# ksalesin/mitsuba3-nasa

Measured on AMD Instinct MI355X. Metric: Msamples/s (pixels×spp/s) fwd + PRB grad, cornell_box 512²; 1/2/4/8 GPU, higher is better.
Workload: dtype f32; 1 GPU; cornell_box 512x512 @ 256 spp/GPU: path fwd (max_depth 8) + prb backward wrt 'white.reflectance.value'; film=512x512, spp_per_gpu=256, spp_total=256

## Files before the change

### mitsuba3-nasa_amd/csrc/mh_wavefront.hip

```cpp
#include <algorithm>
#include <cstdlib>
#include <cmath>
#include <cstring>

#include "mh_shading.hpp"

namespace mh {

struct WfState {
    uint32_t *pd[2];
    float *ox[2], *oy[2], *oz[2], *dx[2], *dy[2], *dz[2], *mt[2];
    float *bx[2], *by[2], *bz[2], *ppx[2], *ppy[2], *ppz[2], *ppdf[2];
    uint64_t *rng[2];
    float *lx[2], *ly[2], *lz[2];
    float *ht, *hu, *hv;
    uint32_t *hp, *hs;
    uint32_t *sid;
    float *sox, *soy, *soz, *sdx, *sdy, *sdz, *smt, *sax, *say, *saz, *sbx, *sby, *sbz;
};

constexpr uint32_t kSeg = 64;
#ifndef MH_SEG_XCD
#define MH_SEG_XCD 0
#endif
// ... 44 lines not shown
        }                                                                                             \
    } while (0)
#define MH_WF_DISPATCH_NR(K, NR, ...)                                                                 \
    do {                                                                                              \
        const dim3 g_(grid), b_(256);                                                                 \
        if (lds && packet) hipLaunchKernelGGL((K<true, true, NR, kEngBvh2>), g_, b_, sh, st, __VA_ARGS__);     \
        else if (lds) hipLaunchKernelGGL((K<true, false, NR, kEngBvh2>), g_, b_, sh, st, __VA_ARGS__);       \
        else if (packet) hipLaunchKernelGGL((K<false, true, NR, kEngBvh2>), g_, b_, sh, st, __VA_ARGS__);    \
        else switch (stream_engine(S)) {                                                              \
            case kEngQuant: hipLaunchKernelGGL((K<false, false, NR, kEngQuant>), g_, b_, sh, st, __VA_ARGS__); break; \
            case kEngWideC: hipLaunchKernelGGL((K<false, false, NR, kEngWideC>), g_, b_, sh, st, __VA_ARGS__); break; \
            case kEngWide: hipLaunchKernelGGL((K<false, false, NR, kEngWide>), g_, b_, sh, st, __VA_ARGS__); break;   \
            default: hipLaunchKernelGGL((K<false, false, NR, kEngBvh2>), g_, b_, sh, st, __VA_ARGS__); break;        \
        }                                                                                             \
    } while (0)

static inline size_t align_up(size_t x) { return (x + 255) & ~size_t(255); }

uint32_t wf_counter_words(uint32_t n_bounces) { return kCtrStride * (n_bounces + 1); }

#ifdef MH_DEBUG
hipError_t guard_read_wf(unsigned long long *out) {
    hipError_t e = hipMemcpyFromSymbol(out, HIP_SYMBOL(g_mh_guard), sizeof(g_mh_guard));
    const unsigned long long z[kGuardCount] = {};
    if (e == hipSuccess) e = hipMemcpyToSymbol(HIP_SYMBOL(g_mh_guard), z, sizeof(z));
    return e;
}
#endif
uint64_t wf_max_chunk() { return 1ull << kPidBits; }

size_t wf_workspace_bytes(uint64_t cap) {
    cap = (cap + kSeg - 1) / kSeg * kSeg;
    return 55 * align_up(cap * 4) + 2 * align_up(cap * 8);
}

static WfState carve(void *ws, uint64_t cap) {
    cap = (cap + kSeg - 1) / kSeg * kSeg;
    uint8_t *p = reinterpret_cast<uint8_t *>(ws);
    auto f = [&]() { float *r = reinterpret_cast<float *>(p); p += align_up(cap * 4); return r; };
    auto u = [&]() { uint32_t *r = reinterpret_cast<uint32_t *>(p); p += align_up(cap * 4); return r; };
    WfState w;
    for (int k = 0; k < 2; ++k) {
        w.pd[k] = u();
        w.ox[k] = f(); w.oy[k] = f(); w.oz[k] = f(); w.dx[k] = f(); w.dy[k] = f(); w.dz[k] = f(); w.mt[k] = f();
        w.bx[k] = f(); w.by[k] = f(); w.bz[k] = f(); w.ppx[k] = f(); w.ppy[k] = f(); w.ppz[k] = f(); w.ppdf[k] = f();
        w.lx[k] = f(); w.ly[k] = f(); w.lz[k] = f();
    }
    w.ht = f(); w.hu = f(); w.hv = f(); w.hp = u(); w.hs = u();
    w.sid = u();
    w.sox = f(); w.soy = f(); w.soz = f(); w.sdx = f(); w.sdy = f(); w.sdz = f(); w.smt = f();
    w.sax = f(); w.say = f(); w.saz = f(); w.sbx = f(); w.sby = f(); w.sbz = f();
    for (int k = 0; k < 2; ++k) {
        w.rng[k] = reinterpret_cast<uint64_t *>(p);
        p += align_up(cap * 8);
    }
    return w;
}

constexpr uint32_t kPkPlanes = 5, kPkExt = 3;
struct WfPacked {
    float4 *base, *ext;
    uint64_t stride;
    uint32_t *tea_base;
    uint64_t tstride;
    MH_DEV float4 *pl(int b, uint32_t k) const { return base + (uint64_t)(b * (int)kPkPlanes + (int)k) * stride; }
    MH_DEV float4 *ex(int b, uint32_t k) const { return ext + (uint64_t)(b * (int)kPkExt + (int)k) * stride; }
    MH_DEV uint32_t *tea(int b) const { return tea_base + (uint64_t)b * tstride; }
};
static WfPacked carve_packed(void *ws, void *ws_ext, uint64_t cap) {
    cap = (cap + kSeg - 1) / kSeg * kSeg;
    WfPacked p;
    p.stride = align_up(cap * 16) / 16;
    p.base = reinterpret_cast<float4 *>(ws);
    p.ext = reinterpret_cast<float4 *>(ws_ext);
    p.tea_base = reinterpret_cast<uint32_t *>(reinterpret_cast<uint8_t *>(ws) + 2 * kPkPlanes * align_up(cap * 16));
    p.tstride = align_up(cap * 4) / 4;
    return p;
}

MH_DEV uint32_t lane_id() { return threadIdx.x & 63u; }

#ifdef MH_EXP_BPHASE
__device__ unsigned long long g_bph[4][12];
#define MH_BPH_DECL uint64_t bph_t = __builtin_amdgcn_s_memtime(); uint64_t bph[12] = {0, 0, 0, 0, 0, 0, 0, 0, 0, 0, 0, 0};
#define MH_BPH(k) do { const uint64_t _t = __builtin_amdgcn_s_memtime(); bph[k] += _t - bph_t; bph_t = _t; } while (0)
#define MH_BPH_ITER() (bph[6] += 1)
#define MH_BPH_FLUSH(grp)                                                                 \
    do {                                                                                  \
        if (lane_id() == 0)                                                               \
            for (int _k = 0; _k < 12; ++_k) atomicAdd(&g_bph[grp][_k], (unsigned long long)bph[_k]); \
    } while (0)
#else
#define MH_BPH_DECL
#define MH_BPH(k) do {} while (0)
#define MH_BPH_ITER() do {} while (0)
#define MH_BPH_FLUSH(grp) do {} while (0)
#endif

struct SegIter {
    uint32_t seg, wave, nwaves;
};
MH_DEV SegIter seg_iter() {
    SegIter it;
#if MH_SEG_XCD
    it.seg = (blockIdx.x & 7u) * 8u + ((blockIdx.x >> 3) & 7u);
#else
    it.seg = blockIdx.x % kSeg;
#endif
    const uint32_t wpb = blockDim.x / 64u;
    it.wave = (blockIdx.x / kSeg) * wpb + threadIdx.x / 64u;
    it.nwaves = (gridDim.x / kSeg) * wpb;
    return it;
}
__host__ __device__ inline uint32_t seg_len(uint64_t n) { return (uint32_t)((n + kSeg - 1) / kSeg); }

MH_DEV uint32_t wave_append(uint32_t *count, bool pred) {
    const unsigned long long m = __ballot(pred);
    const uint32_t tot = (uint32_t)__popcll(m);
    uint32_t base = 0;
    if (lane_id() == 0 && tot) base = atomicAdd(count, tot);
    base = __builtin_amdgcn_readfirstlane(base);
    const uint32_t off = lane_rank(m);
    return base + off;
}

MH_DEV uint64_t pcg_inc(uint32_t seed_value, uint32_t lane) {
    uint32_t v0, v1;
    tea4(seed_value, lane, v0, v1);
    return ((uint64_t)v1 << 1) | 1u;
}

__global__ void __launch_bounds__(256)
k_wf_raygen(DScene S, LaneMap lm, uint32_t seed_value, uint64_t n, uint64_t plane, float *out,
            WfState w, uint32_t *ctr) {
    const uint64_t k = (uint64_t)blockIdx.x * blockDim.x + threadIdx.x;
    if (k < kSeg) {
        const uint64_t L = seg_len(n), b = k * L;
        ctr[k * 32] = b >= n ? 0u : (uint32_t)std::min<uint64_t>(L, n - b);
    }
    if (k >= n) return;
    uint32_t lane, px, py;
    lane_of(lm, k, lane, px, py);
    Pcg rng;
    rng.seed(seed_value, lane);
    float sx = (float)px + rng.next_float(), sy = (float)py + rng.next_float();
    RayT r = camera_ray(S, __builtin_fmaf(sx, S.inv_width, -0.f),
                        __builtin_fmaf(sy, S.inv_height, -0.f));
    w.pd[0][k] = (uint32_t)k;
    w.ox[0][k] = r.o.x; w.oy[0][k] = r.o.y; w.oz[0][k] = r.o.z;
    w.dx[0][k] = r.d.x; w.dy[0][k] = r.d.y; w.dz[0][k] = r.d.z; w.mt[0][k] = r.maxt;
    w.bx[0][k] = 1.f; w.by[0][k] = 1.f; w.bz[0][k] = 1.f;
    w.ppx[0][k] = 0.f; w.ppy[0][k] = 0.f; w.ppz[0][k] = 0.f; w.ppdf[0][k] = 1.f;
    w.rng[0][k] = rng.state;
    w.lx[0][k] = 0.f; w.ly[0][k] = 0.f; w.lz[0][k] = 0.f;
    out[k] = 0.f; out[plane + k] = 0.f; out[2 * plane + k] = 0.f;
    out[3 * plane + k] = sx; out[4 * plane + k] = sy;
}

MH_DEV bool block_has_stride_work(const SegIter &it, uint32_t n) {
    const uint32_t first_wave = (blockIdx.x / kSeg) * (blockDim.x / 64u);
    return first_wave * 64u < n;
}
MH_DEV bool block_has_range_work(const SegIter &it, uint32_t n) {
    const uint32_t first_wave = (blockIdx.x / kSeg) * (blockDim.x / 64u);
    const uint32_t per = (n + it.nwaves - 1) / it.nwaves;
    return first_wave * per < n;
// ... 707 lines not shown
            float rr_prob = fminf(beta_max * (eta * eta), 0.95f);
            bool rr_active = depth >= in.rr_depth;
            if (rr_active) beta = beta * rcp(rr_prob);
            bool rr_continue = rng.next_float() < rr_prob;
            active_next = active_next && (!rr_active || rr_continue);
            if (slot >= 0)
                add_slot(A, slot, prb_indirect_factor(active_next, si, to_local(si, ray.d), bsdf_weight, bs_pdf));
            if (si.valid) depth += 1;
            alive = active_next;
        }
        const uint32_t slot_n = sbase + wave_append(ctr_next + it.seg * 32, alive);
        const uint32_t sslot = sbase + wave_append(ctr + it.seg * 32 + 1, shadow);
        if (alive) {
            w.pd[nxt][slot_n] = pid | (depth << kPidBits);
            w.ox[nxt][slot_n] = ray.o.x; w.oy[nxt][slot_n] = ray.o.y; w.oz[nxt][slot_n] = ray.o.z;
            w.dx[nxt][slot_n] = ray.d.x; w.dy[nxt][slot_n] = ray.d.y; w.dz[nxt][slot_n] = ray.d.z;
            w.mt[nxt][slot_n] = ray.maxt;
            w.bx[nxt][slot_n] = beta.x; w.by[nxt][slot_n] = beta.y; w.bz[nxt][slot_n] = beta.z;
            w.ppx[nxt][slot_n] = prev_p.x; w.ppy[nxt][slot_n] = prev_p.y; w.ppz[nxt][slot_n] = prev_p.z;
            w.ppdf[nxt][slot_n] = prev_pdf;
            w.rng[nxt][slot_n] = rng.state;
            q.dl(nxt, 0)[slot_n] = dL.x; q.dl(nxt, 1)[slot_n] = dL.y; q.dl(nxt, 2)[slot_n] = dL.z;
#pragma unroll
            for (int kk = 0; kk < NR; ++kk)
                if ((uint32_t)kk < n_rgb) {
                    q.A(nxt, kk * 3 + 0)[slot_n] = A[kk][0];
                    q.A(nxt, kk * 3 + 1)[slot_n] = A[kk][1];
                    q.A(nxt, kk * 3 + 2)[slot_n] = A[kk][2];
                }
        }
        if (shadow) {
            w.sox[sslot] = sray.o.x; w.soy[sslot] = sray.o.y; w.soz[sslot] = sray.o.z;
            w.sdx[sslot] = sray.d.x; w.sdy[sslot] = sray.d.y; w.sdz[sslot] = sray.d.z; w.smt[sslot] = sray.maxt;
#pragma unroll
            for (int kk = 0; kk < NR; ++kk)
                if ((uint32_t)kk < n_rgb) {
                    q.G(kk * 3 + 0)[sslot] = G[kk][0];
                    q.G(kk * 3 + 1)[sslot] = G[kk][1];
                    q.G(kk * 3 + 2)[sslot] = G[kk][2];
                }
        }
    }
    flush_partial(acc, q);
}

struct PrbGen {
    uint64_t n_total;
    const float *grad_in;
    int coalesce;
};

struct WfBmp {
    float4 *fin;
    float4 *rec;
    uint32_t *mask[2];
    uint64_t stride;
    uint32_t n_depth;
    int32_t slot;
    MH_DEV float4 *r(uint32_t d, uint32_t k) const { return rec + (uint64_t)(d * 3u + k) * stride; }
};

size_t wf_bmp_workspace_bytes(uint64_t cap, uint32_t n_depth) {
    cap = (cap + kSeg - 1) / kSeg * kSeg;
    return (size_t)(2 + 3 * n_depth) * align_up(cap * 16) + 2 * align_up(cap * 4);
}

static WfBmp carve_bmp(void *ws, uint64_t cap, uint32_t n_depth, int32_t slot) {
    cap = (cap + kSeg - 1) / kSeg * kSeg;
    WfBmp b;
    b.stride = align_up(cap * 16) / 16;
    b.fin = reinterpret_cast<float4 *>(ws);
    b.rec = b.fin + 2 * b.stride;
    uint8_t *m = reinterpret_cast<uint8_t *>(b.rec + (uint64_t)3 * n_depth * b.stride);
    b.mask[0] = reinterpret_cast<uint32_t *>(m);
    b.mask[1] = reinterpret_cast<uint32_t *>(m + align_up(cap * 4));
    b.n_depth = n_depth;
    b.slot = slot;
    return b;
}

#ifndef MH_BOUNCE_BMP_WAVES
#define MH_BOUNCE_BMP_WAVES 4
#endif
template <int NR, bool Gen, bool Bm, bool Det>
__global__ void __launch_bounds__(256, Bm ? MH_BOUNCE_BMP_WAVES : MH_BOUNCE_PRB_WAVES)
k_wf_bounce_prb(DScene S0, IntegratorParams in, LaneMap lm, uint32_t seed_value, WfState w, WfPrb q,
                int cur, uint32_t seg_cap, uint32_t *ctr, uint32_t *ctr_next, PrbGen gen, WfBmp bm, WfDet det) {
    extern __shared__ uint4 lds[];
    const SegIter it = seg_iter();
    auto seg_count = [&](uint32_t sg) -> uint32_t {
        if (Gen) {
            const uint64_t b0 = (uint64_t)sg * seg_cap;
            return b0 >= gen.n_total ? 0u : (uint32_t)std::min<uint64_t>(seg_cap, gen.n_total - b0);
        }
        return __hip_atomic_load(ctr + sg * 32, __ATOMIC_RELAXED, __HIP_MEMORY_SCOPE_AGENT);
    };
    const uint32_t n = seg_count(it.seg);
    if (Gen && blockIdx.x < kSeg && threadIdx.x == 0) ctr[it.seg * 32] = n;
    if (!block_has_stride_work(it, n)) return;
    MH_BPH_DECL
    float *recs = reinterpret_cast<float *>(reinterpret_cast<uint8_t *>(lds) + fused_pairs_offset(S0));
    stage_pair_records(S0, recs);
    const DScene S = stage_tables(S0, lds);
    uint32_t *ws = reinterpret_cast<uint32_t *>(reinterpret_cast<uint8_t *>(lds) + S0.tab_bytes) +
                   (threadIdx.x >> 6) * S0.stack_size;
    uint8_t *dscr = reinterpret_cast<uint8_t *>(lds) + fused_scratch_offset(S0) + (threadIdx.x >> 6) * kDeferScratch;
    uint32_t n_shadow = 0;
    const int nxt = cur ^ 1;
    const uint32_t n_rgb = q.n_rgb;
    float acc[NR][3];
#pragma unroll
    for (int kk = 0; kk < NR; ++kk) acc[kk][0] = acc[kk][1] = acc[kk][2] = 0.f;
    MH_BPH(7);
    const uint32_t seg = it.seg;
    const uint32_t n_iter = (n + it.nwaves * 64u - 1) / (it.nwaves * 64u);
    for (uint32_t itr = 0; itr < n_iter; ++itr) {
        const uint32_t i = (itr * it.nwaves + it.wave) * 64u + lane_id();
        const uint32_t sbase = seg * seg_cap;
        MH_BPH_ITER();
        bool alive = false, shadow = false;
        uint32_t pid = 0, depth = 0;
        RayT ray{v3(0, 0, 0), v3(0, 0, 1), -1.f}, sray{v3(0, 0, 0), v3(0, 0, 1), -1.f};
        V3 beta, prev_p, dL;
        float prev_pdf = 1.f;
        float A[NR][3], G[NR][3];
        float Pp[NR][3];
#pragma unroll
        for (int kk = 0; kk < NR; ++kk) Pp[kk][0] = Pp[kk][1] = Pp[kk][2] = 0.f;
        Pcg rng;
        const uint32_t j = sbase + i;
        MH_GUARD(i >= n || i < seg_cap, kGuardQueueSlot);
        uint64_t gen_state = 0, gen_inc = 0;
        V3 Lrun = v3(0, 0, 0), Le_b = v3(0, 0, 0), Lr_pot = v3(0, 0, 0), D_pot = v3(0, 0, 0), q_ind = v3(0, 0, 0);
        float b_uvx = 0.f, b_uvy = 0.f;
        uint32_t vmask = 0, depth_v = 0;
        bool bvtx = false;
        if (i < n) {
            if (Gen) {
                pid = j;
                uint32_t lane, px, py;
                lane_of(lm, pid, lane, px, py);
                MH_GUARD(px < S0.width && py < S0.height, kGuardPixel);
                Pcg g;
                g.seed(seed_value, lane);
                const float sx = (float)px + g.next_float(), sy = (float)py + g.next_float();
                ray = camera_ray(S0, __builtin_fmaf(sx, S0.inv_width, -0.f),
                                 __builtin_fmaf(sy, S0.inv_height, -0.f));
                gen_state = g.state;
                gen_inc = g.inc;
                dL = gather_dL_wave_lds(S0, gen.coalesce, gen.grad_in, sx, sy, dscr);
            } else {
                const uint32_t pd = w.pd[cur][j];
                pid = pd & kPidMask;
                depth = pd >> kPidBits;
                ray.o = v3(w.ox[cur][j], w.oy[cur][j], w.oz[cur][j]);
                ray.d = v3(w.dx[cur][j], w.dy[cur][j], w.dz[cur][j]);
                ray.maxt = w.mt[cur][j];
            }
            MH_GUARD(pid < gen.n_total, kGuardPathId);
        }
        MH_BPH(0);
        const Hit h = packet_batch<false, true>(S0.nodes, S0.prims, S0.prim_pairs, S0.key_sp, ws, 1u, ray, i < n, recs, dscr);
        MH_BPH(1);
        if (i < n) {
            if (Gen) {
                beta = v3(1.f, 1.f, 1.f);
                prev_p = v3(0.f, 0.f, 0.f);
                prev_pdf = 1.f;
#pragma unroll
                for (int kk = 0; kk < NR; ++kk) A[kk][0] = A[kk][1] = A[kk][2] = 0.f;
                rng.state = gen_state;
            } else {
                const uint32_t jl = j;
                beta = v3(w.bx[cur][jl], w.by[cur][jl], w.bz[cur][jl]);
                prev_p = v3(w.ppx[cur][jl], w.ppy[cur][jl], w.ppz[cur][jl]);
                prev_pdf = w.ppdf[cur][jl];
                dL = v3(q.dl(cur, 0)[jl], q.dl(cur, 1)[jl], q.dl(cur, 2)[jl]);
#pragma unroll
                for (int kk = 0; kk < NR; ++kk)
#pragma unroll
                    for (int c = 0; c < 3; ++c) A[kk][c] = (uint32_t)kk < n_rgb ? q.A(cur, kk * 3 + c)[jl] : 0.f;
                rng.state = w.rng[cur][jl];
                if (Det) {
#pragma unroll
                    for (int kk = 0; kk < NR; ++kk)
#pragma unroll
                        for (int c = 0; c < 3; ++c) Pp[kk][c] = (uint32_t)kk < n_rgb ? det.P(cur, kk * 3 + c)[j] : 0.f;
                }
                if (Bm) {
                    Lrun = v3(w.lx[cur][j], w.ly[cur][j], w.lz[cur][j]);
// ... 41 lines not shown
            if (smooth) rho = tex_eval(S, S.bsdf_tex[b], si.uvx, si.uvy);
            const int32_t slot = smooth ? q.slot_of_tex[S.bsdf_tex[b]] : -1;
            if (Bm) {
                bvtx = slot >= (int32_t)kMaxRgbParams && depth < bm.n_depth;
                depth_v = depth | (bvtx ? (uint32_t)(slot - (int32_t)kMaxRgbParams) << 8 : 0u);
                b_uvx = si.uvx;
                b_uvy = si.uvy;
            }
            if (shadow) {
                V3 wo_em = to_local(si, ds.d);
                V3 bsdf_value_em;
                float bsdf_pdf_em;
                diffuse_eval_pdf(rho, si.wi, wo_em, true, bsdf_value_em, bsdf_pdf_em);
                float mis_em = ds.delta ? 1.f : mis_weight(ds.pdf, bsdf_pdf_em);
                V3 beta_mis_em = beta * mis_em;
                const V3 Lr = (beta_mis_em * bsdf_value_em) * em_weight;
                V3 dLe = dL * Lr;
#pragma unroll
                for (int kk = 0; kk < NR; ++kk) {
                    G[kk][0] = (dLe.x * (A[kk][0] * kInvPi));
                    G[kk][1] = (dLe.y * (A[kk][1] * kInvPi));
                    G[kk][2] = (dLe.z * (A[kk][2] * kInvPi));
                }
                if (slot >= 0 && si.wi.z > 0.f && wo_em.z > 0.f)
                    add_slot(G, slot, (((dL * em_weight) * beta_mis_em) * wo_em.z) * kInvPi);
                if (Bm) {
                    Lr_pot = Lr;
                    if (bvtx && si.wi.z > 0.f && wo_em.z > 0.f)
                        D_pot = (((dL * em_weight) * beta_mis_em) * wo_em.z) * kInvPi;
                }
            }

            (void)rng.next_float();
            float s2x = rng.next_float(), s2y = rng.next_float();
            V3 bs_wo = v3(0, 0, 0), bsdf_weight = v3(0, 0, 0);
            float bs_pdf = 0.f;
            if (smooth && active_next) {
                bs_wo = square_to_cosine_hemisphere(s2x, s2y);
                bs_pdf = kInvPi * bs_wo.z;
                bsdf_weight = (si.wi.z > 0.f && bs_pdf > 0.f) ? rho : v3(0, 0, 0);
            }
            ray = spawn_ray(si.p, si.n, to_world(si, bs_wo));
            beta = beta * bsdf_weight;
            prev_p = si.p;
            prev_pdf = bs_pdf;
            float beta_max = hmax(beta);
            active_next = active_next && beta_max != 0.f;
            float rr_prob = fminf(beta_max * (eta * eta), 0.95f);
            bool rr_active = depth >= in.rr_depth;
            if (rr_active) beta = beta * rcp(rr_prob);
            bool rr_continue = rng.next_float() < rr_prob;
            active_next = active_next && (!rr_active || rr_continue);
            if (slot >= 0) {
                const V3 c = prb_indirect_factor(active_next, si, to_local(si, ray.d), bsdf_weight, bs_pdf);
                add_slot(A, slot, c);
                if (Bm && bvtx) q_ind = c;
            }
            if (si.valid) depth += 1;
            alive = active_next;
        }
        MH_BPH(2);
        const uint32_t slot_n = sbase + wave_append(ctr_next + seg * 32, alive);
        MH_GUARD(!alive || slot_n - sbase < seg_cap, kGuardAppendSlot);
        if (alive) {
            w.pd[nxt][slot_n] = pid | (depth << kPidBits);
            w.ox[nxt][slot_n] = ray.o.x; w.oy[nxt][slot_n] = ray.o.y; w.oz[nxt][slot_n] = ray.o.z;
            w.dx[nxt][slot_n] = ray.d.x; w.dy[nxt][slot_n] = ray.d.y; w.dz[nxt][slot_n] = ray.d.z;
            w.mt[nxt][slot_n] = ray.maxt;
            w.bx[nxt][slot_n] = beta.x; w.by[nxt][slot_n] = beta.y; w.bz[nxt][slot_n] = beta.z;
            w.ppx[nxt][slot_n] = prev_p.x; w.ppy[nxt][slot_n] = prev_p.y; w.ppz[nxt][slot_n] = prev_p.z;
            w.ppdf[nxt][slot_n] = prev_pdf;
            w.rng[nxt][slot_n] = rng.state;
            q.tea(nxt)[slot_n] = (uint32_t)(rng.inc >> 1);
            q.dl(nxt, 0)[slot_n] = dL.x; q.dl(nxt, 1)[slot_n] = dL.y; q.dl(nxt, 2)[slot_n] = dL.z;
#pragma unroll
            for (int kk = 0; kk < NR; ++kk)
                if ((uint32_t)kk < n_rgb) {
                    q.A(nxt, kk * 3 + 0)[slot_n] = A[kk][0];
                    q.A(nxt, kk * 3 + 1)[slot_n] = A[kk][1];
                    q.A(nxt, kk * 3 + 2)[slot_n] = A[kk][2];
                }
        }
        MH_BPH(3);
        const Hit sh = packet_batch<true, true, Gen>(S0.nodes, S0.prims, S0.prim_pairs, S0.key_sp, ws, 1u, sray, shadow, recs, dscr);
        MH_BPH(4);
        const bool unocc = shadow && sh.shape == MH_INVALID;
        if (unocc) {
            float (&ga)[NR][3] = Det ? Pp : acc;
#pragma unroll
            for (int kk = 0; kk < NR; ++kk)
                if ((uint32_t)kk < n_rgb) {
                    ga[kk][0] += G[kk][0];
                    ga[kk][1] += G[kk][1];
                    ga[kk][2] += G[kk][2];
                }
        }
        if (Det && i < n) {
#pragma unroll
            for (int kk = 0; kk < NR; ++kk)
                if ((uint32_t)kk < n_rgb)
#pragma unroll
                    for (int c = 0; c < 3; ++c) {
                        if (alive) det.P(nxt, kk * 3 + c)[slot_n] = Pp[kk][c];
                        else det.fin(kk * 3 + c)[pid] = Pp[kk][c];
                    }
        }
        if (Bm && i < n) {
            Lrun = (Lrun + Le_b) + (unocc ? Lr_pot : v3(0, 0, 0));
            const V3 D = unocc ? D_pot : v3(0, 0, 0);
            if (bvtx && (nonzero(q_ind) || nonzero(D))) {
                const uint32_t dv = depth_v & 0xffu;
                bm.r(dv, 0)[pid] = make_float4(Lrun.x, Lrun.y, Lrun.z, b_uvx);
                bm.r(dv, 1)[pid] = make_float4(q_ind.x, q_ind.y, q_ind.z, b_uvy);
                bm.r(dv, 2)[pid] = make_float4(D.x, D.y, D.z, __uint_as_float(depth_v >> 8));
                vmask |= 1u << dv;
            }
            if (alive) {
                w.lx[nxt][slot_n] = Lrun.x; w.ly[nxt][slot_n] = Lrun.y; w.lz[nxt][slot_n] = Lrun.z;
                bm.mask[nxt][slot_n] = vmask;
            } else {
                bm.fin[pid] = make_float4(Lrun.x, Lrun.y, Lrun.z, __uint_as_float(vmask));
                if (vmask) bm.fin[bm.stride + pid] = make_float4(dL.x, dL.y, dL.z, 0.f);
            }
        }
        n_shadow += (uint32_t)__popcll(__ballot(shadow));
        MH_BPH(5);
    }
    if (lane_id() == 0 && n_shadow) atomicAdd(ctr + it.seg * 32 + 1, n_shadow);
    flush_partial(acc, q);
    if (!Bm && !Det) MH_BPH_FLUSH(Gen ? 2 : 3);
}

struct WfFwdOut {
    float *out;
    uint64_t plane;
    int alpha;
    const int32_t *slot_of_tex;
    float *const *tan;
    const uint32_t *is_rgb;
};

template <bool Gen>
__global__ void __launch_bounds__(256, MH_BOUNCE_PRB_WAVES)
k_wf_bounce_fwd(DScene S0, IntegratorParams in, LaneMap lm, uint32_t seed_value, WfState w, WfPrb q, int cur,
                uint32_t seg_cap, uint32_t *ctr, uint32_t *ctr_next, uint64_t n_total, WfFwdOut fo) {
    extern __shared__ uint4 lds[];
    const SegIter it = seg_iter();
    uint32_t n;
    if (Gen) {
        const uint64_t b0 = (uint64_t)it.seg * seg_cap;
        n = b0 >= n_total ? 0u : (uint32_t)std::min<uint64_t>(seg_cap, n_total - b0);
        if (blockIdx.x < kSeg && threadIdx.x == 0) ctr[it.seg * 32] = n;
    } else {
        n = __hip_atomic_load(ctr + it.seg * 32, __ATOMIC_RELAXED, __HIP_MEMORY_SCOPE_AGENT);
    }
    if (!block_has_stride_work(it, n)) return;
    float *recs = reinterpret_cast<float *>(reinterpret_cast<uint8_t *>(lds) + fused_pairs_offset(S0));
    stage_pair_records(S0, recs);
    const DScene S = stage_tables(S0, lds);
    uint32_t *ws = reinterpret_cast<uint32_t *>(reinterpret_cast<uint8_t *>(lds) + S0.tab_bytes) +
                   (threadIdx.x >> 6) * S0.stack_size;
    uint8_t *dscr = reinterpret_cast<uint8_t *>(lds) + fused_scratch_offset(S0) + (threadIdx.x >> 6) * kDeferScratch;
    GradCtx tg;
    tg.slot_of_tex = fo.slot_of_tex;
    tg.bufs = fo.tan;
    tg.is_rgb = fo.is_rgb;
    uint32_t n_shadow = 0;
    const uint32_t sbase = it.seg * seg_cap;
    const int nxt = cur ^ 1;
    const uint32_t n_iter = (n + it.nwaves * 64u - 1) / (it.nwaves * 64u);
    for (uint32_t itr = 0; itr < n_iter; ++itr) {
        const uint32_t i = (itr * it.nwaves + it.wave) * 64u + lane_id();
        bool alive = false, shadow = false;
        uint32_t pid = 0, depth = 0;
        RayT ray{v3(0, 0, 0), v3(0, 0, 1), -1.f}, sray{v3(0, 0, 0), v3(0, 0, 1), -1.f};
        V3 beta, prev_p, dL = v3(0, 0, 0), T = v3(0, 0, 0), G = v3(0, 0, 0);
        float prev_pdf = 1.f;
        Pcg rng;
        const uint32_t j = sbase + i;
        uint64_t gen_state = 0, gen_inc = 0;
        if (i < n) {
            if (Gen) {
                pid = j;
                uint32_t lane, px, py;
                lane_of(lm, pid, lane, px, py);
                Pcg g;
                g.seed(seed_value, lane);
                const float sx = (float)px + g.next_float(), sy = (float)py + g.next_float();
                ray = camera_ray(S0, __builtin_fmaf(sx, S0.inv_width, -0.f),
                                 __builtin_fmaf(sy, S0.inv_height, -0.f));
                gen_state = g.state;
                gen_inc = g.inc;
                fo.out[3 * fo.plane + pid] = sx;
                fo.out[4 * fo.plane + pid] = sy;
            } else {
                const uint32_t pd = w.pd[cur][j];
                pid = pd & kPidMask;
                depth = pd >> kPidBits;
                ray.o = v3(w.ox[cur][j], w.oy[cur][j], w.oz[cur][j]);
                ray.d = v3(w.dx[cur][j], w.dy[cur][j], w.dz[cur][j]);
                ray.maxt = w.mt[cur][j];
            }
        }
        const Hit h = packet_batch<false, true>(S0.nodes, S0.prims, S0.prim_pairs, S0.key_sp, ws, 1u, ray, i < n, recs, dscr);
        if (i < n) {
            if (Gen) {
                beta = v3(1.f, 1.f, 1.f);
                prev_p = v3(0.f, 0.f, 0.f);
                prev_pdf = 1.f;
// ... 303 lines not shown
}

template <bool InLds, bool Packet, int NR, int Eng>
__global__ void MH_STREAM_LB
k_wf_shadow_prb(DScene S, WfState w, WfPrb q, uint32_t seg_cap, uint32_t *ctr) {
    extern __shared__ uint4 lds[];
    const SegIter it = seg_iter();
    const uint32_t n = __hip_atomic_load(ctr + it.seg * 32 + 1, __ATOMIC_RELAXED, __HIP_MEMORY_SCOPE_AGENT);
    if (!block_has_range_work(it, n)) return;
    LdsBvh B = stage_bvh<InLds && !Packet>(S, lds);
    const uint32_t base = it.seg * seg_cap;
    const uint32_t n_rgb = q.n_rgb;
    float acc[NR][3];
#pragma unroll
    for (int kk = 0; kk < NR; ++kk) acc[kk][0] = acc[kk][1] = acc[kk][2] = 0.f;
    uint32_t r0, r1;
    wave_range(it, n, r0, r1);
    auto load = [&](uint32_t i) {
        const uint32_t j = base + i;
        return RayT{v3(w.sox[j], w.soy[j], w.soz[j]), v3(w.sdx[j], w.sdy[j], w.sdz[j]), w.smt[j]};
    };
    auto store = [&](uint32_t i, const Hit &, bool occluded) {
        if (occluded) return;
        const uint32_t j = base + i;
#pragma unroll
        for (int kk = 0; kk < NR; ++kk)
            if ((uint32_t)kk < n_rgb) {
                acc[kk][0] += q.G(kk * 3 + 0)[j];
                acc[kk][1] += q.G(kk * 3 + 1)[j];
                acc[kk][2] += q.G(kk * 3 + 2)[j];
            }
    };
    if (Packet) trace_packet<true>(S.nodes, S.prims, S.prim_pairs, S.key_sp, B, r0, r1, load, store);
    else trace_stream<true, Eng>(B, r0, r1, load, store);
    flush_partial(acc, q);
}

__global__ void __launch_bounds__(256)
k_wf_grad_reduce(const float *__restrict__ partial, uint32_t grid, float *const *bufs) {
    __shared__ float red[4];
    const uint32_t t = blockIdx.x;
    float s = 0.f;
    for (uint32_t b = threadIdx.x; b < grid; b += blockDim.x) s += partial[(size_t)b * kG + t];
#pragma unroll
    for (int off = 32; off > 0; off >>= 1) s += __shfl_xor(s, off);
    if (lane_id() == 0) red[threadIdx.x >> 6] = s;
    __syncthreads();
    if (threadIdx.x == 0) bufs[t / 3][t % 3] += (red[0] + red[1]) + (red[2] + red[3]);
}

hipError_t launch_wavefront_prb(const DScene &S, const IntegratorParams &in, const LaneMap &lm,
                                uint32_t seed_value, uint64_t n, int coalesce, const float *grad_in,
                                const float *weights, const int32_t *slot_of_tex, uint32_t n_rgb,
                                void *ws, void *ws_prb, uint64_t cap, uint32_t *ctr, uint32_t n_bounces,
                                uint32_t grid, float *partial, hipStream_t st, hipEvent_t *span,
                                const WfBitmapArgs *bmp, void *ws_det) {
    if (n == 0) return hipSuccess;
    if (n > (1ull << kPidBits) || n_bounces > kMaxWfBounces || n_rgb > (uint32_t)kMaxRgbParams) return hipErrorInvalidValue;
    WfState w = carve(ws, cap);
    WfPrb q = carve_prb(ws_prb, cap, partial, slot_of_tex, n_rgb);
    hipError_t e = hipMemsetAsync(ctr, 0, sizeof(uint32_t) * kCtrStride * (n_bounces + 1), st);
    if (e != hipSuccess) return e;
    const bool lds = S.lds_bytes_bvh != 0, packet = use_packet(S);
    const size_t sh = packet ? lds_bytes(S, 256) : stream_lds_bytes(S, 256);
    const uint32_t seg_cap = seg_len(n);
    const bool fused = packet && S.tab_bytes != 0 && !wf_unfused();
    const size_t sh_fused = fused_lds_bytes(S);
    if (S.stack_ovf && (uint64_t)grid * 256 > S.ovf_threads) return hipErrorInvalidValue;
    const bool with_bmp = bmp != nullptr;
    if (with_bmp && (!fused || bmp->n_depth > 31 || bmp->n_depth + 1 < n_bounces || !bmp->ws)) return hipErrorInvalidValue;
    const WfBmp bm = with_bmp ? carve_bmp(bmp->ws, cap, bmp->n_depth, bmp->slot) : WfBmp{};
    const bool det_on = ws_det != nullptr;
    if (det_on && !fused) return hipErrorInvalidValue;
    const WfDet det = det_on ? carve_det(ws_det, cap) : WfDet{};
    if (det_on) {
        e = hipMemsetAsync(det.fin_host(0), 0, (size_t)n_rgb * 3 * det.stride * 4, st);
        if (e != hipSuccess) return e;
    }
    if (!fused)
        hipLaunchKernelGGL(k_wf_raygen_prb, dim3((uint32_t)((n + 255) / 256)), dim3(256), 0, st, S, lm,
                           seed_value, n, coalesce, grad_in, weights, w, q, ctr);
    const PrbGen gen{n, grad_in, coalesce};
    if (span) (void)hipEventRecord(span[0], st);
#define MH_BOUNCE_PRB(NR, GEN, BM, DET)                                                                        \
    hipLaunchKernelGGL((k_wf_bounce_prb<NR, GEN, BM, DET>),                                                    \
                       dim3(grid), dim3(256),      \
                       sh_fused, st, S, in, lm, seed_value, w, q, cur, seg_cap, c, cn, gen, bm, det)
#define MH_BOUNCE_PRB_NR(GEN, BM, DET)                                                                         \
    do {                                                                                                       \
        if (n_rgb <= 1) MH_BOUNCE_PRB(1, GEN, BM, DET);                                                        \
        else MH_BOUNCE_PRB(kMaxRgbParams, GEN, BM, DET);                                                       \
    } while (0)
    for (uint32_t b = 0; b < n_bounces; ++b) {
        uint32_t *c = ctr + kCtrStride * b, *cn = ctr + kCtrStride * (b + 1);
        const int cur = (int)(b & 1);
        if (fused) {
            if (with_bmp && det_on) {
                if (b == 0) MH_BOUNCE_PRB_NR(true, true, true);
                else MH_BOUNCE_PRB_NR(false, true, true);
            } else if (with_bmp) {
                if (b == 0) MH_BOUNCE_PRB_NR(true, true, false);
                else MH_BOUNCE_PRB_NR(false, true, false);
            } else if (det_on) {
                if (b == 0) MH_BOUNCE_PRB_NR(true, false, true);
                else MH_BOUNCE_PRB_NR(false, false, true);
            } else {
                if (b == 0) MH_BOUNCE_PRB_NR(true, false, false);
                else MH_BOUNCE_PRB_NR(false, false, false);
            }
            continue;
        }
        MH_WF_DISPATCH(k_wf_trace, S, w, cur, seg_cap, c);
        if (n_rgb == 1) {
            if (S.tab_bytes)
                hipLaunchKernelGGL((k_wf_shade_prb<true, 1>), dim3(grid), dim3(256), S.tab_bytes, st, S, in, lm,
                                   seed_value, w, q, cur, seg_cap, c, cn);
            else
                hipLaunchKernelGGL((k_wf_shade_prb<false, 1>), dim3(grid), dim3(256), 0, st, S, in, lm, seed_value,
                                   w, q, cur, seg_cap, c, cn);
        } else {
            if (S.tab_bytes)
                hipLaunchKernelGGL((k_wf_shade_prb<true, kMaxRgbParams>), dim3(grid), dim3(256), S.tab_bytes, st, S,
                                   in, lm, seed_value, w, q, cur, seg_cap, c, cn);
            else
                hipLaunchKernelGGL((k_wf_shade_prb<false, kMaxRgbParams>), dim3(grid), dim3(256), 0, st, S, in, lm,
                                   seed_value, w, q, cur, seg_cap, c, cn);
        }
        if (n_rgb == 1) MH_WF_DISPATCH_NR(k_wf_shadow_prb, 1, S, w, q, seg_cap, c);
        else MH_WF_DISPATCH_NR(k_wf_shadow_prb, kMaxRgbParams, S, w, q, seg_cap, c);
    }
#undef MH_BOUNCE_PRB_NR
#undef MH_BOUNCE_PRB
    if (span) (void)hipEventRecord(span[1], st);
    if (with_bmp) {
        const size_t acc_bytes = std::max<size_t>((size_t)bmp->n_floats * kScatAccBytes, 1);
        const bool in_lds = (size_t)bmp->n_floats * 4 <= bmp->lds_max && acc_bytes <= bmp->wg_lds;
        static const int resident = [] {
            int r = 0;
            if (hipOccupancyMaxActiveBlocksPerMultiprocessor(&r, k_wf_bitmap_scatter<true>, kScatThreads, 0) !=
                hipSuccess) {
                (void)hipGetLastError();
                r = 0;
            }
            return r;
        }();
        const uint32_t per_cu = (uint32_t)std::max<size_t>(
            1, std::min<size_t>(resident > 0 ? (size_t)resident : 8u, std::min<size_t>(8, bmp->cu_lds / acc_bytes)));
        const uint32_t blocks = std::max<uint32_t>(1, std::min<uint32_t>(bmp->cus * per_cu, (uint32_t)((n + 4095) / 4096)));
        WfBmpTex bt;
        for (int b = 0; b < kMaxBitmapParams; ++b) { bt.tex[b] = bmp->tex[b]; bt.off[b] = bmp->off[b]; }
        bt.acc64 = bmp->fx_acc;
        bt.fx_max = bmp->fx_word;
        bt.scale = 0.0;
        bt.n_rec = bmp->n_rec;
        const dim3 g_all((uint32_t)((n + 4095) / 4096));
        if (bmp->fx_acc) {
            e = hipMemsetAsync(bmp->fx_word, 0, 4, st);
            if (e != hipSuccess) return e;
            hipLaunchKernelGGL((k_wf_bitmap_scatter<false, 1>), g_all, dim3(256), 0, st, S, bt, bm, (uint32_t)n,
                               bmp->grad, bmp->n_floats);
            uint32_t mb = 0;
            e = hipMemcpyAsync(&mb, bmp->fx_word, 4, hipMemcpyDeviceToHost, st);
            if (e == hipSuccess) e = hipStreamSynchronize(st);
            if (e != hipSuccess) return e;
            float mx;
            memcpy(&mx, &mb, 4);
            int ex = 0;
            if (mx > 0.f && std::isfinite(mx)) (void)std::frexp(mx, &ex);
            bt.scale = std::ldexp(1.0, 31 - ex);
            e = hipMemsetAsync(bmp->fx_acc, 0, (size_t)bmp->n_floats * 8, st);
            if (e != hipSuccess) return e;
            hipLaunchKernelGGL((k_wf_bitmap_scatter<false, 2>), g_all, dim3(256), 0, st, S, bt, bm, (uint32_t)n,
                               bmp->grad, bmp->n_floats);
            hipLaunchKernelGGL(k_fx_fold, dim3(std::max<uint32_t>(1, std::min<uint32_t>(4096, (bmp->n_floats + 255) / 256))),
                               dim3(256), 0, st, reinterpret_cast<const long long *>(bmp->fx_acc), bmp->grad,
                               bmp->n_floats, std::ldexp(1.0, ex - 31));
        } else if (in_lds)
            hipLaunchKernelGGL(k_wf_bitmap_scatter<true>, dim3(blocks), dim3(kScatThreads), (size_t)bmp->n_floats * kScatAccBytes, st, S,
                               bt, bm, (uint32_t)n, bmp->grad, bmp->n_floats);
        else
            hipLaunchKernelGGL(k_wf_bitmap_scatter<false>, dim3((uint32_t)((n + 4095) / 4096)), dim3(256), 0, st, S,
                               bt, bm, (uint32_t)n, bmp->grad, bmp->n_floats);
    }
    if (span) (void)hipEventRecord(span[2], st);
    if (det_on) {
        hipLaunchKernelGGL(k_wf_det_sum, dim3(kDetBlocks), dim3(256), 0, st, det, (uint32_t)(seg_cap * kSeg), n_rgb * 3);
        hipLaunchKernelGGL(k_wf_det_fold, dim3(1), dim3(64), 0, st, det, n_rgb * 3, partial);
    }
    return hipGetLastError();
}

bool wf_fused(const DScene &S) { return use_packet(S) && S.tab_bytes != 0 && !wf_unfused(); }

uint32_t wf_grid(uint32_t grid) { return std::max<uint32_t>(kSeg, grid / kSeg * kSeg); }
uint32_t wf_blocks(int cus, bool shared) {
    uint32_t bpc = shared ? 12 : 30;
    if (const char *e = getenv("MH_WF_BPC")) bpc = std::max(1, atoi(e));
    return (uint32_t)cus * bpc;
}

hipError_t launch_wf_grad_reduce(const float *partial, uint32_t grid, uint32_t n_rgb, float *const *bufs,
                                 hipStream_t st) {
    if (n_rgb == 0) return hipSuccess;
    hipLaunchKernelGGL(k_wf_grad_reduce, dim3(n_rgb * 3), dim3(256), 0, st, partial, grid, bufs);
    return hipGetLastError();
}

#ifdef MH_EXP_BPHASE
extern "C" int mh_exp_bphase(unsigned long long *out, int reset) {
    hipMemcpyFromSymbol(out, HIP_SYMBOL(g_bph), sizeof(g_bph));
    if (reset) {
        unsigned long long z[48] = {0};
        hipMemcpyToSymbol(HIP_SYMBOL(g_bph), z, sizeof(z));
    }
    return 0;
}
#endif
#ifdef MH_EXP_COUNT
extern "C" int mh_exp_counters(unsigned long long *out, int reset) {
    hipMemcpyFromSymbol(out, HIP_SYMBOL(g_exp_cnt), sizeof(g_exp_cnt));
    if (reset) {
        unsigned long long z[32] = {0};
        hipMemcpyToSymbol(HIP_SYMBOL(g_exp_cnt), z, sizeof(z));
    }
    return 0;
}
#endif
}
```

Measured before the change: 2106 Msamples/s.

## Compact shadow rays through a per-wave LDS ring to batch NEE traversal

In the PRB bounce kernel (single-parameter, non-gen, non-bitmap, non-det variant), shadow rays are buffered in a per-wave LDS ring instead of being traced right away with sparse lane occupancy. Traversal runs only when the ring plus new rays would fill a wave, or on the last iteration. Leftover entries are drained after the loop. This is meant to reduce divergent, underfilled shadow-ray traversal, at the cost of extra LDS per block (possible occupancy loss), wave barriers, and added control flow.

```diff
diff --git a/mitsuba3-nasa_amd/csrc/mh_wavefront.hip b/mitsuba3-nasa_amd/csrc/mh_wavefront.hip
--- a/mitsuba3-nasa_amd/csrc/mh_wavefront.hip
+++ b/mitsuba3-nasa_amd/csrc/mh_wavefront.hip
@@ -150,6 +150,7 @@
 
 #ifdef MH_EXP_BPHASE
 __device__ unsigned long long g_bph[4][12];
+static size_t g_prb_ring_lds = 0;
 #define MH_BPH_DECL uint64_t bph_t = __builtin_amdgcn_s_memtime(); uint64_t bph[12] = {0, 0, 0, 0, 0, 0, 0, 0, 0, 0, 0, 0};
 #define MH_BPH(k) do { const uint64_t _t = __builtin_amdgcn_s_memtime(); bph[k] += _t - bph_t; bph_t = _t; } while (0)
 #define MH_BPH_ITER() (bph[6] += 1)
@@ -1023,6 +1024,31 @@
 #ifndef MH_BOUNCE_BMP_WAVES
 #define MH_BOUNCE_BMP_WAVES 4
 #endif
+#ifndef MH_PRB_NEE_RING
+#define MH_PRB_NEE_RING 1
+#endif
+constexpr uint32_t kNeeRingFields = 10;
+constexpr uint32_t kNeeRingFloats = kNeeRingFields * 64u;
+template <int NR, bool Gen, bool Bm, bool Det>
+constexpr bool prb_nee_ring() { return MH_PRB_NEE_RING && NR == 1 && !Gen && !Bm && !Det; }
+MH_DEV void nee_ring_put(float *ring, uint32_t slot, const RayT &r, const float (&g)[3]) {
+    ring[0 * 64 + slot] = r.o.x; ring[1 * 64 + slot] = r.o.y; ring[2 * 64 + slot] = r.o.z;
+    ring[3 * 64 + slot] = r.d.x; ring[4 * 64 + slot] = r.d.y; ring[5 * 64 + slot] = r.d.z;
+    ring[6 * 64 + slot] = r.maxt;
+    ring[7 * 64 + slot] = g[0]; ring[8 * 64 + slot] = g[1]; ring[9 * 64 + slot] = g[2];
+}
+MH_DEV void nee_ring_get(const float *ring, uint32_t slot, RayT &r, float (&g)[3]) {
+    r.o = v3(ring[0 * 64 + slot], ring[1 * 64 + slot], ring[2 * 64 + slot]);
+    r.d = v3(ring[3 * 64 + slot], ring[4 * 64 + slot], ring[5 * 64 + slot]);
+    r.maxt = ring[6 * 64 + slot];
+    g[0] = ring[7 * 64 + slot]; g[1] = ring[8 * 64 + slot]; g[2] = ring[9 * 64 + slot];
+}
+MH_DEV void nee_ring_sync() {
+    __builtin_amdgcn_fence(__ATOMIC_RELEASE, "wavefront");
+    __builtin_amdgcn_wave_barrier();
+    __builtin_amdgcn_fence(__ATOMIC_ACQUIRE, "wavefront");
+}
+
 template <int NR, bool Gen, bool Bm, bool Det>
 __global__ void __launch_bounds__(256, Bm ? MH_BOUNCE_BMP_WAVES : MH_BOUNCE_PRB_WAVES)
 k_wf_bounce_prb(DScene S0, IntegratorParams in, LaneMap lm, uint32_t seed_value, WfState w, WfPrb q,
@@ -1047,6 +1073,12 @@
                    (threadIdx.x >> 6) * S0.stack_size;
     uint8_t *dscr = reinterpret_cast<uint8_t *>(lds) + fused_scratch_offset(S0) + (threadIdx.x >> 6) * kDeferScratch;
     uint32_t n_shadow = 0;
+    constexpr bool Ring = prb_nee_ring<NR, Gen, Bm, Det>();
+    float *ring = nullptr;
+    if constexpr (Ring)
+        ring = reinterpret_cast<float *>(reinterpret_cast<uint8_t *>(lds) + fused_lds_bytes(S0)) +
+               __builtin_amdgcn_readfirstlane(threadIdx.x >> 6) * kNeeRingFloats;
+    uint32_t ring_n = 0;
     const int nxt = cur ^ 1;
     const uint32_t n_rgb = q.n_rgb;
     float acc[NR][3];
@@ -1254,6 +1286,26 @@
                 }
         }
         MH_BPH(3);
+        if constexpr (Ring) {
+            const unsigned long long sm = __ballot(shadow);
+            const uint32_t k = (uint32_t)__popcll(sm);
+            n_shadow += k;
+            if (ring_n + k < 64u && itr + 1u != n_iter) {
+                if (shadow) nee_ring_put(ring, ring_n + lane_rank(sm), sray, G[0]);
+                ring_n += k;
+                MH_BPH(4);
+                MH_BPH(5);
+                continue;
+            }
+            const uint32_t take = std::min(ring_n, 64u - k), fr = lane_rank(~sm);
+            nee_ring_sync();
+            if (!shadow && fr < take) {
+                nee_ring_get(ring, ring_n - 1u - fr, sray, G[0]);
+                shadow = true;
+            }
+            ring_n -= take;
+            nee_ring_sync();
+        }
         const Hit sh = packet_batch<true, true, Gen>(S0.nodes, S0.prims, S0.prim_pairs, S0.key_sp, ws, 1u, sray, shadow, recs, dscr);
         MH_BPH(4);
         const bool unocc = shadow && sh.shape == MH_INVALID;
@@ -1295,8 +1347,25 @@
                 if (vmask) bm.fin[bm.stride + pid] = make_float4(dL.x, dL.y, dL.z, 0.f);
             }
         }
-        n_shadow += (uint32_t)__popcll(__ballot(shadow));
+        if constexpr (!Ring) n_shadow += (uint32_t)__popcll(__ballot(shadow));
         MH_BPH(5);
+    }
+    if constexpr (Ring) {
+        while (ring_n) {
+            const uint32_t take = std::min(ring_n, 64u);
+            const bool has = lane_id() < take;
+            RayT sray{v3(0, 0, 0), v3(0, 0, 1), -1.f};
+            float g[3] = {0.f, 0.f, 0.f};
+            nee_ring_sync();
+            if (has) nee_ring_get(ring, ring_n - 1u - lane_id(), sray, g);
+            ring_n -= take;
+            const Hit sh = packet_batch<true, true, false>(S0.nodes, S0.prims, S0.prim_pairs, S0.key_sp, ws, 1u, sray, has, recs, dscr);
+            if (has && sh.shape == MH_INVALID && n_rgb) {
+                acc[0][0] += g[0];
+                acc[0][1] += g[1];
+                acc[0][2] += g[2];
+            }
+        }
     }
     if (lane_id() == 0 && n_shadow) atomicAdd(ctr + it.seg * 32 + 1, n_shadow);
     flush_partial(acc, q);
@@ -1766,10 +1835,13 @@
                            seed_value, n, coalesce, grad_in, weights, w, q, ctr);
     const PrbGen gen{n, grad_in, coalesce};
     if (span) (void)hipEventRecord(span[0], st);
+#ifdef MH_EXP_BPHASE
+    g_prb_ring_lds = sh_fused + (prb_nee_ring<1, false, false, false>() ? 4u * kNeeRingFloats * 4u : 0u);
+#endif
 #define MH_BOUNCE_PRB(NR, GEN, BM, DET)                                                                        \
     hipLaunchKernelGGL((k_wf_bounce_prb<NR, GEN, BM, DET>),                                                    \
                        dim3(grid), dim3(256),      \
-                       sh_fused, st, S, in, lm, seed_value, w, q, cur, seg_cap, c, cn, gen, bm, det)
+                       sh_fused + (prb_nee_ring<NR, GEN, BM, DET>() ? 4u * kNeeRingFloats * 4u : 0u), st, S, in, lm, seed_value, w, q, cur, seg_cap, c, cn, gen, bm, det)
 #define MH_BOUNCE_PRB_NR(GEN, BM, DET)                                                                         \
     do {                                                                                                       \
         if (n_rgb <= 1) MH_BOUNCE_PRB(1, GEN, BM, DET);                                                        \
@@ -1891,6 +1963,13 @@
 }
 
 #ifdef MH_EXP_BPHASE
+extern "C" int mh_exp_prb_occupancy(unsigned long long *lds_bytes) {
+    int r = -1;
+    if (lds_bytes) *lds_bytes = g_prb_ring_lds;
+    if (hipOccupancyMaxActiveBlocksPerMultiprocessor(&r, k_wf_bounce_prb<1, false, false, false>, 256, g_prb_ring_lds) != hipSuccess)
+        return -1;
+    return r;
+}
 extern "C" int mh_exp_bphase(unsigned long long *out, int reset) {
     hipMemcpyFromSymbol(out, HIP_SYMBOL(g_bph), sizeof(g_bph));
     if (reset) {
```

New measurement: 2143 Msamples/s (median of 6 runs). +1.7%, better.
